# kubeai-project/kubeai

Measured on AMD Instinct MI355X. Metric: output_tokens_per_s (k6 multi-turn chat), higher is better.
Workload: dtype fp8; 1 GPU; model=llama-3-8b, global_batch=40, seq_len=8192, parallelism=dp1, prefix_cache=True

## Files before the change

kubeai_amd/csrc/bindings.cpp:

```cpp
#include <torch/extension.h>

#include <utility>

#include "attention_plan.h"

void rmsnorm(torch::Tensor out, torch::Tensor x, torch::Tensor weight,
             double eps);
void fused_add_rmsnorm(torch::Tensor x, torch::Tensor residual,
                       torch::Tensor weight, double eps);
void rope(torch::Tensor q, torch::Tensor k, torch::Tensor positions,
          torch::Tensor cos_sin);
void rope_and_cache(torch::Tensor q, torch::Tensor k, torch::Tensor v,
                    torch::Tensor positions, torch::Tensor cos_sin,
                    torch::Tensor k_cache, torch::Tensor v_cache,
                    torch::Tensor slot_mapping);
void reshape_and_cache(torch::Tensor k, torch::Tensor v, torch::Tensor k_cache,
                       torch::Tensor v_cache, torch::Tensor slot_mapping);
void paged_attention_decode(torch::Tensor out, torch::Tensor q,
                            torch::Tensor k_cache, torch::Tensor v_cache,
                            torch::Tensor block_tables, torch::Tensor seq_lens,
                            double scale, int64_t window, double softcap);
void paged_attention_decode_fp8(torch::Tensor out, torch::Tensor out_fp8,
                                torch::Tensor out_scale, torch::Tensor q,
                                torch::Tensor k_cache, torch::Tensor v_cache,
// ... 14 lines not shown
                             torch::Tensor seq_lens, double scale,
                             int64_t window, double softcap);
void silu_and_mul(torch::Tensor out, torch::Tensor x);
void gelu_and_mul(torch::Tensor out, torch::Tensor x);
void skinny_gemm(torch::Tensor y, torch::Tensor x, torch::Tensor w);
void int4_dequant(torch::Tensor out, torch::Tensor qp, torch::Tensor sp,
                  torch::Tensor zp, int64_t N, int64_t K, int64_t group);
void int4_gemm(torch::Tensor y, torch::Tensor x, torch::Tensor qp,
               torch::Tensor sp, torch::Tensor zp, int64_t N, int64_t K,
               int64_t group);
int64_t int4_gemm_tiles(int64_t N, int64_t M);
void greedy_sample(torch::Tensor out, torch::Tensor logits);
void gumbel_sample(torch::Tensor out, torch::Tensor logits,
                   torch::Tensor temperature, torch::Tensor seeds,
                   int64_t step);
void sgmv(torch::Tensor y, torch::Tensor x, torch::Tensor A, torch::Tensor B,
          torch::Tensor idx, double scale);
void register_chwbl(pybind11::module_& m);
pybind11::bytes xgmi_alloc();
void xgmi_connect(int64_t rank, int64_t world,
                  const std::vector<pybind11::bytes>& handles);
void xgmi_fused_allreduce_add_rmsnorm(torch::Tensor x, torch::Tensor residual,
                                      torch::Tensor weight, double eps);
int64_t xgmi_error_count();
int64_t xgmi_max_elems();
void xgmi_shutdown();
void rmsnorm_fp8(torch::Tensor out, torch::Tensor out_scale, torch::Tensor x,
                 torch::Tensor weight, double eps);
void fused_add_rmsnorm_fp8(torch::Tensor out, torch::Tensor out_scale,
                           torch::Tensor x, torch::Tensor residual,
                           torch::Tensor weight, double eps);
void silu_and_mul_fp8(torch::Tensor out, torch::Tensor out_scale,
                      torch::Tensor x);
void quant_fp8(torch::Tensor out, torch::Tensor out_scale, torch::Tensor x);
void nucleus_stats(torch::Tensor m, torch::Tensor z, torch::Tensor logits,
                   torch::Tensor temps);
void nucleus_accept(torch::Tensor ok, torch::Tensor logits,
                    torch::Tensor cand, torch::Tensor m, torch::Tensor z,
                    torch::Tensor temps, torch::Tensor top_ps,
                    torch::Tensor top_ks);

static std::pair<int64_t, int64_t> prefill_plan(int64_t Tq, int64_t B,
                                                int64_t n_q, int64_t n_kv,
                                                int64_t hd, int64_t max_blocks,
                                                int64_t window,
                                                double softcap) {
  TORCH_CHECK(n_kv > 0 && n_q % n_kv == 0);
  const attn_plan::PrefillPlan p = attn_plan::prefill_plan(
      Tq, (int)B, (int)n_q, (int)n_kv, (int)hd, (int)max_blocks, window,
// ... 32 lines not shown
        "decode attention kernel (q, k, v are only read)");
  m.def("paged_attention_prefill", &paged_attention_prefill,
        "paged causal flash attention over cached KV");
  m.def("gelu_and_mul", &gelu_and_mul, "GeGLU tanh-gelu(gate)*up");
  m.def("silu_and_mul", &silu_and_mul, "SwiGLU activation");
  m.def("skinny_gemm", &skinny_gemm, "weight-streaming GEMM for M<=64");
  m.def("int4_dequant", &int4_dequant,
        "packed int4 weight -> bf16 [N, K], bit-equal to Int4Weight.dequant()");
  m.def("int4_gemm", &int4_gemm,
        "fused dequant + GEMM over a packed int4 weight, M <= 64");
  m.def("int4_gemm_tiles", &int4_gemm_tiles,
        "16-column tiles per workgroup int4_gemm launches with",
        pybind11::arg("N"), pybind11::arg("M"));
  m.def("greedy_sample", &greedy_sample, "argmax sampling");
  m.def("gumbel_sample", &gumbel_sample, "temperature sampling (hash RNG)");
  m.def("rmsnorm_fp8", &rmsnorm_fp8, "rmsnorm with fused fp8 row quant");
  m.def("fused_add_rmsnorm_fp8", &fused_add_rmsnorm_fp8,
        "residual add + rmsnorm with fused fp8 row quant");
  m.def("silu_and_mul_fp8", &silu_and_mul_fp8, "SwiGLU with fused fp8 quant");
  m.def("quant_fp8", &quant_fp8, "bf16 -> fp8 row quant");
  m.def("nucleus_stats", &nucleus_stats, "per-row softmax max + Z");
  m.def("nucleus_accept", &nucleus_accept,
        "nucleus membership of sampled tokens (mass above < p, rank < k)");
  m.def("xgmi_alloc", &xgmi_alloc, "allocate + export the IPC comm buffer");
  m.def("xgmi_connect", &xgmi_connect, "open peer IPC buffers");
  m.def("xgmi_fused_allreduce_add_rmsnorm", &xgmi_fused_allreduce_add_rmsnorm,
        "one-shot xGMI all-reduce fused with residual add + RMSNorm");
  m.def("xgmi_error_count", &xgmi_error_count, "spin-wait timeout count");
  m.def("xgmi_max_elems", &xgmi_max_elems, "one-shot capacity (bf16 elems)");
  m.def("xgmi_shutdown", &xgmi_shutdown, "free/close comm buffers");
  m.def("sgmv", &sgmv, "segmented gather LoRA apply (one adapter segment)");
  register_chwbl(m);
}
```

kubeai_amd/csrc/common.h:

```cpp
#pragma once

#include <hip/hip_runtime.h>
#include <hip/hip_bf16.h>
#include <hip/hip_fp16.h>
#include <hip/hip_fp8.h>
#include <stdint.h>
#include <c10/hip/HIPStream.h>

#define WAVE_SIZE 64
#define DEV_INLINE __device__ __forceinline__

typedef __hip_bfloat16 bf16_t;

typedef ushort __attribute__((ext_vector_type(8))) ushort8;
typedef ushort __attribute__((ext_vector_type(4))) ushort4_t;
typedef float __attribute__((ext_vector_type(4))) float4_t;

DEV_INLINE float bf16_to_f32(ushort u) {
  union {
    uint32_t i;
    float f;
  } c;
  c.i = ((uint32_t)u) << 16;
  return c.f;
// ... 126 lines not shown
#pragma unroll
  for (int j = 0; j < 4; ++j) {
    packed[j].x = f32_to_fp8(f[2 * j] * inv_scale);
    packed[j].y = f32_to_fp8(f[2 * j + 1] * inv_scale);
  }
  return *reinterpret_cast<uint2*>(packed);
}

DEV_INLINE float row_scale_fp8(const float amax, float* smem,
                               float* __restrict__ scale_out) {
  const float gmax = fmaxf(block_amax(amax, smem), 1e-6f);
  if (threadIdx.x == 0) *scale_out = gmax / 448.0f;
  return 448.0f / gmax;
}

DEV_INLINE float silu(const float x) { return x / (1.0f + __expf(-x)); }

DEV_INLINE uint64_t splitmix64(uint64_t z) {
  z += 0x9e3779b97f4a7c15ull;
  z = (z ^ (z >> 30)) * 0xbf58476d1ce4e5b9ull;
  z = (z ^ (z >> 27)) * 0x94d049bb133111ebull;
  return z ^ (z >> 31);
}

DEV_INLINE float hash_uniform(uint64_t key, uint64_t idx) {
  uint64_t h = splitmix64(key ^ (idx * 0xd1342543de82ef95ull));
  uint32_t m = (uint32_t)(h >> 40);
  return ((float)m + 1.0f) * (1.0f / 16777216.0f);
}

// ... 9 lines not shown
```

kubeai_amd/csrc/row_kernels.hip:

```cpp
#include <torch/extension.h>

#include <type_traits>

#include "common.h"
#include "dispatch.h"

namespace {

constexpr int kBlock = 256;
constexpr int kBlockWide = 512;
constexpr int kMaxIters = 8;
constexpr int kMaxH = kBlockWide * 8 * kMaxIters;

template <int kThreads, int kIters>
DEV_INLINE void store_row_fp8(unsigned char* __restrict__ orow,
                              const float (&vals)[kIters][8],
                              const float inv_scale, const int nvec) {
#pragma unroll
  for (int it = 0; it < kIters; ++it) {
    const int i = threadIdx.x + it * kThreads;
    if (i < nvec)
      *reinterpret_cast<uint2*>(orow + i * 8) = quant8_fp8(vals[it], inv_scale);
  }
}

template <bool kFused, bool kFp8Out, int kThreads, int kIters>
__launch_bounds__(kThreads) __global__ void rmsnorm_kernel(
    std::conditional_t<kFp8Out, unsigned char, ushort>* __restrict__ out,
    float* __restrict__ out_scale,
    ushort* __restrict__ x,
    ushort* __restrict__ residual,
    const ushort* __restrict__ w,
    const float eps, const int H) {
  const int row = blockIdx.x;
  ushort8* xrow = reinterpret_cast<ushort8*>(x + (int64_t)row * H);
  ushort8* rrow =
      kFused ? reinterpret_cast<ushort8*>(residual + (int64_t)row * H) : nullptr;
// ... 77 lines not shown
    for (int j = 0; j < 8; ++j) v[j] = bf16_to_f32(xv[j]);
  }
};

struct LoadSwiglu {
  static constexpr int kInWidth = 2;
  DEV_INLINE static void load(const ushort* __restrict__ in, const int W,
                              const int i, float (&v)[8]) {
    const ushort8 g = reinterpret_cast<const ushort8*>(in)[i];
    const ushort8 u = reinterpret_cast<const ushort8*>(in + W)[i];
#pragma unroll
    for (int j = 0; j < 8; ++j) v[j] = silu(bf16_to_f32(g[j])) * bf16_to_f32(u[j]);
  }
};

template <typename Producer, int kThreads, int kIters>
__launch_bounds__(kThreads) __global__ void row_fp8_kernel(
    unsigned char* __restrict__ out,
    float* __restrict__ out_scale,
    const ushort* __restrict__ xin,
    const int W) {
  const int row = blockIdx.x;
  const ushort* in = xin + (int64_t)row * Producer::kInWidth * W;
  const int nvec = W / 8;

  float vals[kIters][8];
  float amax = 0.f;
#pragma unroll
  for (int it = 0; it < kIters; ++it) {
    const int i = threadIdx.x + it * kThreads;
    if (i < nvec) {
      Producer::load(in, W, i, vals[it]);
#pragma unroll
      for (int j = 0; j < 8; ++j) amax = fmaxf(amax, fabsf(vals[it][j]));
    }
  }
  __shared__ float red[16];
  const float inv_scale = row_scale_fp8(amax, red, out_scale + row);
  store_row_fp8<kThreads, kIters>(out + (int64_t)row * W, vals, inv_scale, nvec);
}

enum class RowPolicy { kNorm, kMax };

template <RowPolicy kPolicy, typename Launch>
void dispatch_row(const int nvec, Launch&& launch) {
  if (nvec <= kBlock) {
    launch(Int<kBlock>{}, Int<1>{});
  } else if (nvec <= kBlock * 2) {
    launch(Int<kBlock>{}, Int<2>{});
  } else if (nvec <= kBlock * 4) {
    launch(Int<kBlock>{}, Int<4>{});
  } else if constexpr (kPolicy == RowPolicy::kNorm) {
    if (nvec <= kBlock * kMaxIters) launch(Int<kBlock>{}, Int<kMaxIters>{});
    else launch(Int<kBlockWide>{}, Int<kMaxIters>{});
// ... 16 lines not shown
  check_row_op(x, H);
  const int T = x.numel() / H;
  using out_t = std::conditional_t<kFp8Out, unsigned char, ushort>;
  dispatch_row<RowPolicy::kNorm>(H / 8, [&](auto threads, auto iters) {
    constexpr int kThreads = decltype(threads)::value;
    constexpr int kIters = decltype(iters)::value;
    hipLaunchKernelGGL((rmsnorm_kernel<kFused, kFp8Out, kThreads, kIters>),
                       dim3(T), dim3(kThreads), 0,
                       c10::hip::getCurrentHIPStream().stream(), (out_t*)out,
                       out_scale, (ushort*)x.data_ptr(), (ushort*)residual,
                       (const ushort*)weight.data_ptr(), (float)eps, H);
  });
  HIP_CHECK_KERNEL();
}

template <typename Producer>
void launch_row_fp8(torch::Tensor& out, torch::Tensor& out_scale,
                    const torch::Tensor& x) {
  const int W = x.size(-1) / Producer::kInWidth;
  check_row_op(x, W);
  TORCH_CHECK(x.size(-1) == (int64_t)W * Producer::kInWidth);
  const int T = x.numel() / x.size(-1);
  if (T == 0) return;
  dispatch_row<RowPolicy::kMax>(W / 8, [&](auto threads, auto iters) {
    constexpr int kThreads = decltype(threads)::value;
    constexpr int kIters = decltype(iters)::value;
    hipLaunchKernelGGL((row_fp8_kernel<Producer, kThreads, kIters>), dim3(T),
                       dim3(kThreads), 0,
                       c10::hip::getCurrentHIPStream().stream(),
                       (unsigned char*)out.data_ptr(),
                       out_scale.data_ptr<float>(),
                       (const ushort*)x.data_ptr(), W);
  });
  HIP_CHECK_KERNEL();
}

}

void rmsnorm(torch::Tensor out, torch::Tensor x, torch::Tensor weight,
             double eps) {
  TORCH_CHECK(out.is_contiguous());
  launch_rmsnorm<false, false>(out.data_ptr(), nullptr, x, nullptr, weight, eps);
// ... 16 lines not shown
                           torch::Tensor x, torch::Tensor residual,
                           torch::Tensor weight, double eps) {
  TORCH_CHECK(residual.is_contiguous());
  launch_rmsnorm<true, true>(out.data_ptr(), out_scale.data_ptr<float>(), x,
                             residual.data_ptr(), weight, eps);
}

void silu_and_mul_fp8(torch::Tensor out, torch::Tensor out_scale,
                      torch::Tensor x) {
  launch_row_fp8<LoadSwiglu>(out, out_scale, x);
}

void quant_fp8(torch::Tensor out, torch::Tensor out_scale, torch::Tensor x) {
  launch_row_fp8<LoadBf16>(out, out_scale, x);
}
```

kubeai_amd/csrc/sampling.hip:

```cpp
#include <torch/extension.h>

#include "common.h"

namespace {

constexpr int kBlock = 256;
constexpr int kSplits = 32;

template <bool kGumbel>
__global__ void sample_stage1(
    float* __restrict__ part_val,
    int32_t* __restrict__ part_idx,
    const float* __restrict__ logits,
    const float* __restrict__ temperature,
    const int64_t* __restrict__ seeds,
    const int64_t step, const int V) {
  const int b = blockIdx.x;
  const int split = blockIdx.y;
  const int chunk = (V + kSplits - 1) / kSplits;
  const int lo = split * chunk;
  const int hi = min(V, lo + chunk);
  const float* row = logits + (int64_t)b * V;
  float temp = 1.0f;
  uint64_t key = 0;
  bool greedy = !kGumbel;
  if constexpr (kGumbel) {
    temp = temperature[b];
    if (temp <= 0.f) greedy = true;
    key = (uint64_t)seeds[b] * 1000003ull + (uint64_t)step;
  }

  float best = -INFINITY;
  int best_idx = V;
  for (int v = lo + threadIdx.x; v < hi; v += kBlock) {
    float val = row[v];
    if (!greedy) {
      float u = hash_uniform(key, (uint64_t)v);
      val = val / temp + (-__logf(-__logf(u)));
    }
    if (val > best || (val == best && v < best_idx)) {
      best = val;
      best_idx = v;
    }
  }
#pragma unroll
  for (int off = 32; off > 0; off >>= 1) {
    float ov = __shfl_xor(best, off, 64);
    int oi = __shfl_xor(best_idx, off, 64);
    if (ov > best || (ov == best && oi < best_idx)) {
      best = ov;
      best_idx = oi;
    }
  }
  __shared__ float sval[4];
  __shared__ int sidx[4];
  const int wave = threadIdx.x / WAVE_SIZE;
  if (threadIdx.x % WAVE_SIZE == 0) {
    sval[wave] = best;
    sidx[wave] = best_idx;
  }
  __syncthreads();
  if (threadIdx.x == 0) {
#pragma unroll
    for (int w = 1; w < kBlock / WAVE_SIZE; ++w) {
      if (sval[w] > best || (sval[w] == best && sidx[w] < best_idx)) {
        best = sval[w];
        best_idx = sidx[w];
      }
    }
    part_val[b * kSplits + split] = best;
    part_idx[b * kSplits + split] = best_idx;
  }
}

__global__ void sample_stage2(int64_t* __restrict__ out,
                              const float* __restrict__ part_val,
                              const int32_t* __restrict__ part_idx) {
  const int b = blockIdx.x;
  const int lane = threadIdx.x;
  float best = (lane < kSplits) ? part_val[b * kSplits + lane] : -INFINITY;
  int best_idx = (lane < kSplits) ? part_idx[b * kSplits + lane] : INT32_MAX;
#pragma unroll
  for (int off = 32; off > 0; off >>= 1) {
    float ov = __shfl_xor(best, off, 64);
    int oi = __shfl_xor(best_idx, off, 64);
    if (ov > best || (ov == best && oi < best_idx)) {
      best = ov;
      best_idx = oi;
    }
  }
  if (lane == 0) out[b] = best_idx;
}

template <bool kGumbel>
void launch_sample(torch::Tensor out, torch::Tensor logits,
                   const float* temp_ptr, const int64_t* seed_ptr,
                   int64_t step) {
  const int B = logits.size(0), V = logits.size(1);
  if (B == 0) return;
  auto opts = torch::TensorOptions().device(logits.device());
  auto part_val = torch::empty({B, kSplits}, opts.dtype(torch::kFloat32));
  auto part_idx = torch::empty({B, kSplits}, opts.dtype(torch::kInt32));
  auto stream = c10::hip::getCurrentHIPStream().stream();
  hipLaunchKernelGGL((sample_stage1<kGumbel>), dim3(B, kSplits), dim3(kBlock),
                     0, stream, part_val.data_ptr<float>(),
                     part_idx.data_ptr<int32_t>(), logits.data_ptr<float>(),
                     temp_ptr, seed_ptr, step, V);
  HIP_CHECK_KERNEL();
  hipLaunchKernelGGL(sample_stage2, dim3(B), dim3(WAVE_SIZE), 0, stream,
                     out.data_ptr<int64_t>(), part_val.data_ptr<float>(),
                     part_idx.data_ptr<int32_t>());
  HIP_CHECK_KERNEL();
}

}

void greedy_sample(torch::Tensor out, torch::Tensor logits) {
  TORCH_CHECK(logits.is_contiguous());
  TORCH_CHECK(logits.scalar_type() == torch::kFloat32,
              "sampling expects fp32 logits");
  launch_sample<false>(out, logits, nullptr, nullptr, 0);
}

void gumbel_sample(torch::Tensor out, torch::Tensor logits,
                   torch::Tensor temperature, torch::Tensor seeds,
                   int64_t step) {
  TORCH_CHECK(logits.is_contiguous());
  TORCH_CHECK(logits.scalar_type() == torch::kFloat32);
  TORCH_CHECK(temperature.scalar_type() == torch::kFloat32);
  TORCH_CHECK(seeds.scalar_type() == torch::kInt64);
  launch_sample<true>(out, logits, temperature.data_ptr<float>(),
                      seeds.data_ptr<int64_t>(), step);
}


namespace {

__global__ void nucleus_stats_kernel(
    float* __restrict__ m_out, float* __restrict__ z_out,
    const float* __restrict__ logits, const float* __restrict__ temps,
    const int V) {
  const int row = blockIdx.x;
  const float* x = logits + (int64_t)row * V;
  const float t = fmaxf(temps[row], 1e-6f);
  __shared__ float red[16];
  float m = -INFINITY;
  for (int i = threadIdx.x; i < V; i += blockDim.x) m = fmaxf(m, x[i]);
// ... 88 lines not shown
```

kubeai_amd/engine/quant.py:

```python
from __future__ import annotations

import torch
import torch.nn as nn

FP8_DTYPE = torch.float8_e4m3fn
FP8_MAX = 448.0


class Fp8Linear(nn.Module):

    def __init__(self, weight_bf16: torch.Tensor, bias: torch.Tensor | None = None):
        super().__init__()
        if bias is not None:
            self.register_buffer("bias", bias.detach().to(torch.bfloat16))
        else:
            self.bias = None
        w = weight_bf16.detach().float()
        w_amax = w.abs().amax(dim=1, keepdim=True).clamp_min(1e-6)
        w_scale = w_amax / FP8_MAX
        wq = (w / w_scale).clamp(-FP8_MAX, FP8_MAX).to(FP8_DTYPE)
        self.register_buffer("weight_fp8", wq.contiguous())
        self.register_buffer("weight_scale", w_scale.reshape(1, -1).contiguous())
        self.out_features, self.in_features = weight_bf16.shape

# ... 7 lines not shown
        if not xq.is_cuda:
            x = xq.float() * x_scale.view(-1, 1)
            w = self.weight_fp8.float() * self.weight_scale.reshape(-1, 1)
            y = (x @ w.t()).to(torch.bfloat16)
            return y + self.bias if self.bias is not None else y
        return torch._scaled_mm(
            xq,
            self.weight_fp8.t(),
            scale_a=x_scale.view(-1, 1),
            scale_b=self.weight_scale,
            bias=self.bias,
            out_dtype=torch.bfloat16,
        )

    def forward(self, x: torch.Tensor) -> torch.Tensor:
        a_amax = x.float().abs().amax(dim=-1, keepdim=True).clamp_min(1e-6)
        a_scale = a_amax / FP8_MAX
        xq = (x.float() / a_scale).clamp(-FP8_MAX, FP8_MAX).to(FP8_DTYPE)
        if not x.is_cuda:
            return self.forward_quantized(xq, a_scale.squeeze(-1))
        return torch._scaled_mm(
            xq,
            self.weight_fp8.t(),
            scale_a=a_scale,
            scale_b=self.weight_scale,
            bias=self.bias,
            out_dtype=torch.bfloat16,
        )


_TARGETS = ("qkv_proj", "o_proj", "gate_up_proj", "down_proj", "lm_head")


# ... 19 lines not shown
```

kubeai_amd/engine/runner.py:

```python
from __future__ import annotations

import os
from typing import Optional

import torch

from kubeai_amd import ops
from kubeai_amd.models.config import ModelArchConfig
from kubeai_amd.models.llama import LlamaForCausalLM

from .batch import ForwardBatch
from .scheduler import SchedulerOutput


class _DecodeGraph:

    def __init__(self, runner: "ModelRunner", b_pad: int, bt_max: int):
        dev = runner.device
        self.b_pad = b_pad
        self.bt_max = bt_max
        self.input_ids = torch.zeros(b_pad, dtype=torch.int32, device=dev)
        self.positions = torch.zeros(b_pad, dtype=torch.int32, device=dev)
        self.slots = torch.full((b_pad,), -1, dtype=torch.int64, device=dev)
        self.block_tables = torch.zeros(
            (b_pad, bt_max), dtype=torch.int32, device=dev
        )
        self.seq_lens = torch.ones(b_pad, dtype=torch.int32, device=dev)
        logits_idx = torch.arange(b_pad, dtype=torch.int64, device=dev)
        self.fb = ForwardBatch(
            input_ids=self.input_ids,
            positions=self.positions,
            slot_mapping=self.slots,
            n_decode=b_pad,
            decode_block_tables=self.block_tables,
            decode_seq_lens=self.seq_lens,
            n_prefill=0,
            prefill_query_start_loc=None,
            prefill_seq_lens=None,
            prefill_block_tables=None,
            logits_indices=logits_idx,
        )
        torch.cuda.synchronize()
        for _ in range(2):
            h = runner.model(self.fb)
            runner.model.compute_logits(h[logits_idx])
        torch.cuda.synchronize()
        self.graph = torch.cuda.CUDAGraph()
        with torch.cuda.graph(self.graph):
            h = runner.model(self.fb)
            self.logits = runner.model.compute_logits(h[logits_idx])

    def run(self, input_ids, positions, slots, tables, seq_lens) -> torch.Tensor:
        b = len(input_ids)
        self.input_ids[:b].copy_(input_ids, non_blocking=True)
        self.positions[:b].copy_(positions, non_blocking=True)
        self.slots[:b].copy_(slots, non_blocking=True)
        if b < self.b_pad:
            self.slots[b:].fill_(-1)
            self.seq_lens[b:].fill_(1)
            self.block_tables[b:].fill_(0)
        self.block_tables[:b, : tables.shape[1]].copy_(tables, non_blocking=True)
        if tables.shape[1] < self.bt_max:
            self.block_tables[:b, tables.shape[1] :].fill_(0)
        self.seq_lens[:b].copy_(seq_lens, non_blocking=True)
        self.graph.replay()
        return self.logits[:b]


class ModelRunner:
    def __init__(
        self,
        arch: ModelArchConfig,
        device: str = "cuda",
        dtype: torch.dtype = torch.bfloat16,
        block_size: int = 16,
        num_gpu_blocks: Optional[int] = None,
        gpu_memory_utilization: float = 0.90,
        seed: int = 0,
        tp_group=None,
# ... 286 lines not shown
            self._graphs[b_pad] = g
        bs = self.block_size
        ids, pos, slots, lens = [], [], [], []
        import numpy as np

        tables = np.zeros((b, g.bt_max), dtype=np.int32)
        for i, ss in enumerate(out.decode):
            req = ss.req
            t = ss.chunk_start
            ids.append(req.tokens[t])
            pos.append(t)
            slots.append(req.block_table[t // bs] * bs + t % bs)
            lens.append(t + 1)
            bt = req.block_table
            tables[i, : len(bt)] = bt
        return g.run(
            torch.tensor(ids, dtype=torch.int32),
            torch.tensor(pos, dtype=torch.int32),
            torch.tensor(slots, dtype=torch.int64),
            torch.from_numpy(tables),
            torch.tensor(lens, dtype=torch.int32),
        )

    @torch.inference_mode()
    def execute(self, out: SchedulerOutput, step: int) -> dict[str, int]:
        logits = None
        if (
            self.enable_graphs
            and not out.prefill
            and out.decode
            and not (
                getattr(self, "lora_manager", None) is not None
                and self.lora_manager.active
            )
        ):
            logits = self._execute_graph(out)
        if logits is None:
# ... 35 lines not shown
            if r.params.logit_bias:
                for t, b in r.params.logit_bias.items():
                    if 0 <= t < V:
                        rows.append(i)
                        cols.append(t)
                        vals.append(b)
        if rows:
            flat = torch.tensor(
                [ri * V + ci for ri, ci in zip(rows, cols)],
                dtype=torch.int64, device=dev_l,
            )
            logits.view(-1).scatter_add_(
                0, flat, torch.tensor(vals, dtype=logits.dtype, device=dev_l)
            )
        temps = [r.params.temperature for r in sample_reqs]
        if all(t <= 0.0 for t in temps):
            tokens = ops.greedy_sample(logits.contiguous())
        else:
            needs_topk = any(
                (r.params.top_p < 1.0 or r.params.top_k > 0)
                and r.params.temperature > 0
                for r in sample_reqs
            )
            dev = self.device
            t_t = torch.tensor(temps, dtype=torch.float32, device=dev)
            seeds = torch.tensor(
                [
                    r.params.seed if r.params.seed is not None else _seed_of(r.request_id)
                    for r in sample_reqs
                ],
                dtype=torch.int64,
                device=dev,
            )
            if needs_topk:
                tokens = _sample_topk_topp(
                    logits,
                    [r.params.top_p for r in sample_reqs],
                    [r.params.top_k for r in sample_reqs],
                    [r.params.temperature for r in sample_reqs],
                    t_t, seeds, step,
                    cache=self._sampling_cache,
                ).to(dev)
            else:
                tokens = ops.gumbel_sample(logits.contiguous(), t_t, seeds, step)
        tokens = tokens.cpu().tolist()
        if any(r.params.json_mode for r in sample_reqs):
            tokens = self._constrain_json(sample_reqs, tokens, logits)
        tokens_t = torch.tensor(tokens, dtype=torch.int64, device=logits.device)
        lse = torch.logsumexp(logits, dim=-1)
        chosen = logits.gather(1, tokens_t.view(-1, 1)).squeeze(1)
        logprobs = (chosen - lse).cpu().tolist()
        self.last_logprobs = {
            r.request_id: float(lp) for r, lp in zip(sample_reqs, logprobs)
        }
        self.last_top_logprobs = {}
        want = max((r.params.logprobs for r in sample_reqs), default=0)
        if want > 0:
            k = min(want, logits.shape[-1])
            tv, ti = (logits - lse.unsqueeze(1)).topk(k, dim=-1)
            tv, ti = tv.cpu().tolist(), ti.cpu().tolist()
            for r, vs, ids in zip(sample_reqs, tv, ti):
                if r.params.logprobs > 0:
                    n = r.params.logprobs
                    self.last_top_logprobs[r.request_id] = [
                        (int(i), float(v)) for i, v in zip(ids[:n], vs[:n])
                    ]
# ... 217 lines not shown
```

kubeai_amd/ops/__init__.py:

```python
from __future__ import annotations

import os

import torch

from . import ref

_C = None
_C_IMPORT_ERROR: Exception | None = None
try:
    from kubeai_amd import _C
except Exception as e:
    _C_IMPORT_ERROR = e


def have_hip_ext() -> bool:
    return _C is not None


def _require_ext() -> None:
    if _C is None:
        raise RuntimeError(
            "kubeai_amd HIP extension (kubeai_amd._C) is not built but a GPU "
            "tensor reached the ops layer. Build it with "
# ... 275 lines not shown
    T, two_i = x.shape
    out, scale = _empty_fp8_rows((T, two_i // 2), x.device)
    _C.silu_and_mul_fp8(out, scale, x)
    return out, scale


def quant_fp8(x):
    if not x.is_cuda:
        return ref.quant_fp8(x)
    _require_ext()
    out, scale = _empty_fp8_rows(x.shape, x.device)
    _C.quant_fp8(out, scale, x)
    return out, scale


def greedy_sample(logits):
    if logits.is_cuda:
        _require_ext()
        out = torch.empty(logits.shape[0], dtype=torch.int64, device=logits.device)
        _C.greedy_sample(out, logits)
        return out
    return ref.greedy_sample(logits)


def gumbel_sample(logits, temperature, seeds, step: int):
    if logits.is_cuda:
        _require_ext()
        out = torch.empty(logits.shape[0], dtype=torch.int64, device=logits.device)
        _C.gumbel_sample(out, logits, temperature, seeds, step)
        return out
    return ref.gumbel_sample(logits, temperature, seeds, step)


def nucleus_stats(logits, temps):
    if logits.is_cuda:
        _require_ext()
        S = logits.shape[0]
        m = torch.empty(S, dtype=torch.float32, device=logits.device)
        z = torch.empty_like(m)
        _C.nucleus_stats(m, z, logits, temps)
        return m, z
    t = temps.clamp_min(1e-6).unsqueeze(1)
    m = logits.max(dim=-1).values
    z = torch.exp((logits - m.unsqueeze(1)) / t).sum(-1)
    return m, z

# ... 16 lines not shown
```

kubeai_amd/ops/ref.py:

```python
from __future__ import annotations

import math

import torch



def rmsnorm(x: torch.Tensor, weight: torch.Tensor, eps: float) -> torch.Tensor:
    xf = x.float()
    var = xf.pow(2).mean(dim=-1, keepdim=True)
    y = xf * torch.rsqrt(var + eps) * weight.float()
    return y.to(x.dtype)


def fused_add_rmsnorm(
    x: torch.Tensor, residual: torch.Tensor, weight: torch.Tensor, eps: float
) -> tuple[torch.Tensor, torch.Tensor]:
    res = (x.float() + residual.float())
    y = rmsnorm(res, weight, eps)
    return y.to(x.dtype), res.to(x.dtype)



def make_cos_sin_cache(
# ... 227 lines not shown
    B, V = lf.shape
    out = torch.empty(B, dtype=torch.int64, device=logits.device)
    idx = torch.arange(V)
    for b in range(B):
        t = float(temperature[b])
        if t <= 0.0:
            out[b] = int(lf[b].argmax())
            continue
        key = (int(seeds[b]) * 1000003 + step) & _U64
        u = hash_uniform(key, idx).to(lf.device)
        g = -torch.log(-torch.log(u))
        out[b] = int((lf[b] / t + g).argmax())
    return out


def topk_topp_sample(
    logits: torch.Tensor,
    temperature: torch.Tensor,
    top_p: torch.Tensor,
    top_k: torch.Tensor,
    seeds: torch.Tensor,
    step: int,
) -> torch.Tensor:
    lf = logits.float()
    B, V = lf.shape
    out = torch.empty(B, dtype=torch.int64, device=logits.device)
    for b in range(B):
        t = float(temperature[b])
        if t <= 0.0:
            out[b] = int(lf[b].argmax())
# ... 9 lines not shown
        sp, si = sp[keep], si[keep]
        gen = torch.Generator(device="cpu")
        gen.manual_seed(int(seeds[b]) * 1000003 + step)
        r = float(torch.rand((), generator=gen)) * float(sp.sum())
        idx = int(torch.searchsorted(sp.cumsum(0), torch.tensor(r)).clamp(max=sp.shape[0] - 1))
        out[b] = int(si[idx])
    return out


def quant_fp8(x: torch.Tensor):
    xf = x.float()
    amax = xf.abs().amax(dim=-1).clamp_min(1e-6)
    scale = amax / 448.0
    q = (xf / scale[:, None]).clamp(-448.0, 448.0).to(torch.float8_e4m3fn)
    return q, scale
```

Before: 7380 tok/s.

## Fuse sampling with logprob/logsumexp, add div-form fp8 quant kernel, stage graph inputs

Sampling kernels now also compute the row logsumexp and the chosen token's logprob, so the separate torch logsumexp, gather and extra device-to-host copy after sampling are gone. Tokens and logprobs are packed into one buffer and copied to the host together. A division-form fp8 row-quant kernel is added for Fp8Linear, and the decode graph inputs are staged through a pinned host buffer with a single copy. These cut per-step launches and host syncs, at the cost of more kernel variants and added complexity.

```diff
diff --git a/kubeai_amd/csrc/bindings.cpp b/kubeai_amd/csrc/bindings.cpp
--- a/kubeai_amd/csrc/bindings.cpp
+++ b/kubeai_amd/csrc/bindings.cpp
@@ -52,6 +52,14 @@
 void gumbel_sample(torch::Tensor out, torch::Tensor logits,
                    torch::Tensor temperature, torch::Tensor seeds,
                    int64_t step);
+void greedy_sample_logprob(torch::Tensor out, torch::Tensor out_logprob,
+                           torch::Tensor out_lse, torch::Tensor logits);
+void gumbel_sample_logprob(torch::Tensor out, torch::Tensor out_logprob,
+                           torch::Tensor out_lse, torch::Tensor logits,
+                           torch::Tensor temperature, torch::Tensor seeds,
+                           int64_t step);
+void token_logprobs(torch::Tensor out_logprob, torch::Tensor out_lse,
+                    torch::Tensor logits, torch::Tensor tokens);
 void sgmv(torch::Tensor y, torch::Tensor x, torch::Tensor A, torch::Tensor B,
           torch::Tensor idx, double scale);
 void register_chwbl(pybind11::module_& m);
@@ -71,6 +79,8 @@
 void silu_and_mul_fp8(torch::Tensor out, torch::Tensor out_scale,
                       torch::Tensor x);
 void quant_fp8(torch::Tensor out, torch::Tensor out_scale, torch::Tensor x);
+void quant_fp8_div(torch::Tensor out, torch::Tensor out_scale,
+                   torch::Tensor x);
 void nucleus_stats(torch::Tensor m, torch::Tensor z, torch::Tensor logits,
                    torch::Tensor temps);
 void nucleus_accept(torch::Tensor ok, torch::Tensor logits,
@@ -133,11 +143,19 @@
         pybind11::arg("N"), pybind11::arg("M"));
   m.def("greedy_sample", &greedy_sample, "argmax sampling");
   m.def("gumbel_sample", &gumbel_sample, "temperature sampling (hash RNG)");
+  m.def("greedy_sample_logprob", &greedy_sample_logprob,
+        "argmax sampling + the token's logprob and the row logsumexp");
+  m.def("gumbel_sample_logprob", &gumbel_sample_logprob,
+        "temperature sampling + the token's logprob and the row logsumexp");
+  m.def("token_logprobs", &token_logprobs,
+        "logprob of given tokens and the row logsumexp, one launch");
   m.def("rmsnorm_fp8", &rmsnorm_fp8, "rmsnorm with fused fp8 row quant");
   m.def("fused_add_rmsnorm_fp8", &fused_add_rmsnorm_fp8,
         "residual add + rmsnorm with fused fp8 row quant");
   m.def("silu_and_mul_fp8", &silu_and_mul_fp8, "SwiGLU with fused fp8 quant");
   m.def("quant_fp8", &quant_fp8, "bf16 -> fp8 row quant");
+  m.def("quant_fp8_div", &quant_fp8_div,
+        "bf16 -> fp8 row quant, division form (Fp8Linear.forward)");
   m.def("nucleus_stats", &nucleus_stats, "per-row softmax max + Z");
   m.def("nucleus_accept", &nucleus_accept,
         "nucleus membership of sampled tokens (mass above < p, rank < k)");
diff --git a/kubeai_amd/csrc/common.h b/kubeai_amd/csrc/common.h
--- a/kubeai_amd/csrc/common.h
+++ b/kubeai_amd/csrc/common.h
@@ -164,6 +164,26 @@
   return 448.0f / gmax;
 }
 
+DEV_INLINE float row_scale_fp8_div(const float amax, float* smem,
+                                   float* __restrict__ scale_out) {
+  const float gmax = fmaxf(block_amax(amax, smem), 1e-6f);
+  const float scale = gmax * (float)(1.0 / 448.0);
+  if (threadIdx.x == 0) *scale_out = scale;
+  return scale;
+}
+
+DEV_INLINE uint2 quant8_fp8_div(const float (&f)[8], const float scale) {
+  uchar2 packed[4];
+#pragma unroll
+  for (int j = 0; j < 4; ++j) {
+    packed[j].x =
+        f32_to_fp8(fminf(fmaxf(f[2 * j] / scale, -448.0f), 448.0f));
+    packed[j].y =
+        f32_to_fp8(fminf(fmaxf(f[2 * j + 1] / scale, -448.0f), 448.0f));
+  }
+  return *reinterpret_cast<uint2*>(packed);
+}
+
 DEV_INLINE float silu(const float x) { return x / (1.0f + __expf(-x)); }
 
 DEV_INLINE uint64_t splitmix64(uint64_t z) {
diff --git a/kubeai_amd/csrc/row_kernels.hip b/kubeai_amd/csrc/row_kernels.hip
--- a/kubeai_amd/csrc/row_kernels.hip
+++ b/kubeai_amd/csrc/row_kernels.hip
@@ -12,15 +12,16 @@
 constexpr int kMaxIters = 8;
 constexpr int kMaxH = kBlockWide * 8 * kMaxIters;
 
-template <int kThreads, int kIters>
+template <int kThreads, int kIters, bool kDiv = false>
 DEV_INLINE void store_row_fp8(unsigned char* __restrict__ orow,
                               const float (&vals)[kIters][8],
-                              const float inv_scale, const int nvec) {
+                              const float factor, const int nvec) {
 #pragma unroll
   for (int it = 0; it < kIters; ++it) {
     const int i = threadIdx.x + it * kThreads;
     if (i < nvec)
-      *reinterpret_cast<uint2*>(orow + i * 8) = quant8_fp8(vals[it], inv_scale);
+      *reinterpret_cast<uint2*>(orow + i * 8) =
+          kDiv ? quant8_fp8_div(vals[it], factor) : quant8_fp8(vals[it], factor);
   }
 }
 
@@ -128,7 +129,7 @@
   }
 };
 
-template <typename Producer, int kThreads, int kIters>
+template <typename Producer, bool kDiv, int kThreads, int kIters>
 __launch_bounds__(kThreads) __global__ void row_fp8_kernel(
     unsigned char* __restrict__ out,
     float* __restrict__ out_scale,
@@ -150,8 +151,10 @@
     }
   }
   __shared__ float red[16];
-  const float inv_scale = row_scale_fp8(amax, red, out_scale + row);
-  store_row_fp8<kThreads, kIters>(out + (int64_t)row * W, vals, inv_scale, nvec);
+  const float factor = kDiv ? row_scale_fp8_div(amax, red, out_scale + row)
+                            : row_scale_fp8(amax, red, out_scale + row);
+  store_row_fp8<kThreads, kIters, kDiv>(out + (int64_t)row * W, vals, factor,
+                                        nvec);
 }
 
 enum class RowPolicy { kNorm, kMax };
@@ -198,7 +201,7 @@
   HIP_CHECK_KERNEL();
 }
 
-template <typename Producer>
+template <typename Producer, bool kDiv = false>
 void launch_row_fp8(torch::Tensor& out, torch::Tensor& out_scale,
                     const torch::Tensor& x) {
   const int W = x.size(-1) / Producer::kInWidth;
@@ -209,7 +212,7 @@
   dispatch_row<RowPolicy::kMax>(W / 8, [&](auto threads, auto iters) {
     constexpr int kThreads = decltype(threads)::value;
     constexpr int kIters = decltype(iters)::value;
-    hipLaunchKernelGGL((row_fp8_kernel<Producer, kThreads, kIters>), dim3(T),
+    hipLaunchKernelGGL((row_fp8_kernel<Producer, kDiv, kThreads, kIters>), dim3(T),
                        dim3(kThreads), 0,
                        c10::hip::getCurrentHIPStream().stream(),
                        (unsigned char*)out.data_ptr(),
@@ -256,3 +259,8 @@
 void quant_fp8(torch::Tensor out, torch::Tensor out_scale, torch::Tensor x) {
   launch_row_fp8<LoadBf16>(out, out_scale, x);
 }
+
+void quant_fp8_div(torch::Tensor out, torch::Tensor out_scale,
+                   torch::Tensor x) {
+  launch_row_fp8<LoadBf16, true>(out, out_scale, x);
+}
diff --git a/kubeai_amd/csrc/sampling.hip b/kubeai_amd/csrc/sampling.hip
--- a/kubeai_amd/csrc/sampling.hip
+++ b/kubeai_amd/csrc/sampling.hip
@@ -1,20 +1,50 @@
 #include <torch/extension.h>
 
 #include "common.h"
+#include "dispatch.h"
 
 namespace {
 
 constexpr int kBlock = 256;
+constexpr int kWaves = kBlock / WAVE_SIZE;
 constexpr int kSplits = 32;
-
-template <bool kGumbel>
-__global__ void sample_stage1(
-    float* __restrict__ part_val,
-    int32_t* __restrict__ part_idx,
+constexpr int kRegIters = 16;
+
+DEV_INLINE float max_waves(const float (&s)[kWaves]) {
+  return fmaxf(fmaxf(s[0], s[1]), fmaxf(s[2], s[3]));
+}
+
+DEV_INLINE float sum_waves(const float (&s)[kWaves]) {
+  return ((s[0] + s[1]) + s[2]) + s[3];
+}
+static_assert(kWaves == 4, "max_waves / sum_waves spell four waves");
+
+DEV_INLINE float exp_ref(const float m) { return m == -INFINITY ? 0.f : m; }
+
+DEV_INLINE float merge_lse(const float m, const float s) {
+  const float M = wave_reduce_max(m);
+  const float t = (m == -INFINITY) ? 0.f : s * expf(m - M);
+  float S = 0.f;
+#pragma unroll
+  for (int i = 0; i < kSplits; ++i) S += __shfl(t, i, 64);
+  return logf(S) + M;
+}
+
+struct SamplePartials {
+  float* val;
+  int32_t* idx;
+  float* m;
+  float* s;
+};
+
+template <bool kGumbel, bool kLse, bool kRegs>
+__launch_bounds__(kBlock) __global__ void sample_stage1(
+    const SamplePartials part,
     const float* __restrict__ logits,
     const float* __restrict__ temperature,
     const int64_t* __restrict__ seeds,
     const int64_t step, const int V) {
+  static_assert(kLse || !kRegs, "registers serve the second sweep only");
   const int b = blockIdx.x;
   const int split = blockIdx.y;
   const int chunk = (V + kSplits - 1) / kSplits;
@@ -32,8 +62,9 @@
 
   float best = -INFINITY;
   int best_idx = V;
-  for (int v = lo + threadIdx.x; v < hi; v += kBlock) {
-    float val = row[v];
+  float m = -INFINITY;
+  auto visit = [&](const int v, const float raw) {
+    float val = raw;
     if (!greedy) {
       float u = hash_uniform(key, (uint64_t)v);
       val = val / temp + (-__logf(-__logf(u)));
@@ -42,6 +73,22 @@
       best = val;
       best_idx = v;
     }
+    if constexpr (kLse) m = fmaxf(m, raw);
+  };
+  float x[kRegs ? kRegIters : 1];
+  if constexpr (kRegs) {
+#pragma unroll
+    for (int it = 0; it < kRegIters; ++it) {
+      const int v = lo + threadIdx.x + it * kBlock;
+      x[it] = v < hi ? row[v] : -INFINITY;
+    }
+#pragma unroll
+    for (int it = 0; it < kRegIters; ++it) {
+      const int v = lo + threadIdx.x + it * kBlock;
+      if (v < hi) visit(v, x[it]);
+    }
+  } else {
+    for (int v = lo + threadIdx.x; v < hi; v += kBlock) visit(v, row[v]);
   }
 #pragma unroll
   for (int off = 32; off > 0; off >>= 1) {
@@ -52,34 +99,64 @@
       best_idx = oi;
     }
   }
-  __shared__ float sval[4];
-  __shared__ int sidx[4];
+  if constexpr (kLse) m = wave_reduce_max(m);
+  __shared__ float sval[kWaves];
+  __shared__ int sidx[kWaves];
+  __shared__ float smax[kWaves];
+  __shared__ float ssum[kWaves];
   const int wave = threadIdx.x / WAVE_SIZE;
   if (threadIdx.x % WAVE_SIZE == 0) {
     sval[wave] = best;
     sidx[wave] = best_idx;
+    if constexpr (kLse) smax[wave] = m;
   }
   __syncthreads();
   if (threadIdx.x == 0) {
 #pragma unroll
-    for (int w = 1; w < kBlock / WAVE_SIZE; ++w) {
+    for (int w = 1; w < kWaves; ++w) {
       if (sval[w] > best || (sval[w] == best && sidx[w] < best_idx)) {
         best = sval[w];
         best_idx = sidx[w];
       }
     }
-    part_val[b * kSplits + split] = best;
-    part_idx[b * kSplits + split] = best_idx;
-  }
-}
-
+    part.val[b * kSplits + split] = best;
+    part.idx[b * kSplits + split] = best_idx;
+  }
+  if constexpr (kLse) {
+    m = max_waves(smax);
+    const float ref = exp_ref(m);
+    float s = 0.f;
+    if constexpr (kRegs) {
+#pragma unroll
+      for (int it = 0; it < kRegIters; ++it) {
+        const int v = lo + threadIdx.x + it * kBlock;
+        if (v < hi) s += expf(x[it] - ref);
+      }
+    } else {
+      for (int v = lo + threadIdx.x; v < hi; v += kBlock)
+        s += expf(row[v] - ref);
+    }
+    s = wave_reduce_sum(s);
+    if (threadIdx.x % WAVE_SIZE == 0) ssum[wave] = s;
+    __syncthreads();
+    if (threadIdx.x == 0) {
+      part.m[b * kSplits + split] = m;
+      part.s[b * kSplits + split] = sum_waves(ssum);
+    }
+  }
+}
+
+template <bool kLse>
 __global__ void sample_stage2(int64_t* __restrict__ out,
-                              const float* __restrict__ part_val,
-                              const int32_t* __restrict__ part_idx) {
+                              float* __restrict__ out_logprob,
+                              float* __restrict__ out_lse,
+                              const SamplePartials part,
+                              const float* __restrict__ logits,
+                              const int V) {
   const int b = blockIdx.x;
   const int lane = threadIdx.x;
-  float best = (lane < kSplits) ? part_val[b * kSplits + lane] : -INFINITY;
-  int best_idx = (lane < kSplits) ? part_idx[b * kSplits + lane] : INT32_MAX;
+  float best = (lane < kSplits) ? part.val[b * kSplits + lane] : -INFINITY;
+  int best_idx = (lane < kSplits) ? part.idx[b * kSplits + lane] : INT32_MAX;
 #pragma unroll
   for (int off = 32; off > 0; off >>= 1) {
     float ov = __shfl_xor(best, off, 64);
@@ -89,48 +166,178 @@
       best_idx = oi;
     }
   }
+  if constexpr (kLse) {
+    const float lse =
+        merge_lse((lane < kSplits) ? part.m[b * kSplits + lane] : -INFINITY,
+                  (lane < kSplits) ? part.s[b * kSplits + lane] : 0.f);
+    if (lane == 0) {
+      const float xt =
+          best_idx < V ? logits[(int64_t)b * V + best_idx] : (float)NAN;
+      out_logprob[b] = xt - lse;
+      out_lse[b] = lse;
+    }
+  }
   if (lane == 0) out[b] = best_idx;
 }
 
-template <bool kGumbel>
-void launch_sample(torch::Tensor out, torch::Tensor logits,
-                   const float* temp_ptr, const int64_t* seed_ptr,
-                   int64_t step) {
+constexpr int kGroups = 4;
+static_assert(kSplits % kGroups == 0, "every group runs every round");
+
+__launch_bounds__(kBlock* kGroups) __global__ void token_logprobs_kernel(
+    float* __restrict__ out_logprob,
+    float* __restrict__ out_lse,
+    const float* __restrict__ logits,
+    const int64_t* __restrict__ tokens,
+    const int V) {
+  const int b = blockIdx.x;
+  const int g = threadIdx.x / kBlock;
+  const int tid = threadIdx.x % kBlock;
+  const int wave = tid / WAVE_SIZE;
+  const float* row = logits + (int64_t)b * V;
+  const int chunk = (V + kSplits - 1) / kSplits;
+  __shared__ float smax[kGroups][kWaves];
+  __shared__ float ssum[kGroups][kWaves];
+  __shared__ float pm[kSplits];
+  __shared__ float ps[kSplits];
+  for (int r = 0; r < kSplits / kGroups; ++r) {
+    const int split = r * kGroups + g;
+    const int lo = split * chunk;
+    const int hi = min(V, lo + chunk);
+    float m = -INFINITY;
+    for (int v = lo + tid; v < hi; v += kBlock) m = fmaxf(m, row[v]);
+    m = wave_reduce_max(m);
+    if (tid % WAVE_SIZE == 0) smax[g][wave] = m;
+    __syncthreads();
+    m = max_waves(smax[g]);
+    const float ref = exp_ref(m);
+    float s = 0.f;
+    for (int v = lo + tid; v < hi; v += kBlock) s += expf(row[v] - ref);
+    s = wave_reduce_sum(s);
+    if (tid % WAVE_SIZE == 0) ssum[g][wave] = s;
+    __syncthreads();
+    if (tid == 0) {
+      pm[split] = m;
+      ps[split] = sum_waves(ssum[g]);
+    }
+  }
+  __syncthreads();
+  if (threadIdx.x < WAVE_SIZE) {
+    const int lane = threadIdx.x;
+    const float lse = merge_lse((lane < kSplits) ? pm[lane] : -INFINITY,
+                                (lane < kSplits) ? ps[lane] : 0.f);
+    if (lane == 0) {
+      const int64_t t = tokens[b];
+      const float xt = (t >= 0 && t < V) ? row[t] : (float)NAN;
+      out_logprob[b] = xt - lse;
+      out_lse[b] = lse;
+    }
+  }
+}
+
+void check_logits(const torch::Tensor& logits) {
+  TORCH_CHECK(logits.dim() == 2 && logits.is_contiguous());
+  TORCH_CHECK(logits.scalar_type() == torch::kFloat32,
+              "sampling expects fp32 logits");
+}
+
+template <typename T>
+T* row_output(const torch::Tensor& t, const torch::Tensor& logits) {
+  TORCH_CHECK(t.is_contiguous() && t.numel() == logits.size(0) &&
+              t.device() == logits.device());
+  return t.data_ptr<T>();
+}
+
+template <bool kGumbel, bool kLse>
+void launch_sample(int64_t* out, float* out_logprob, float* out_lse,
+                   const torch::Tensor& logits, const float* temp_ptr,
+                   const int64_t* seed_ptr, int64_t step) {
   const int B = logits.size(0), V = logits.size(1);
   if (B == 0) return;
-  auto opts = torch::TensorOptions().device(logits.device());
-  auto part_val = torch::empty({B, kSplits}, opts.dtype(torch::kFloat32));
-  auto part_idx = torch::empty({B, kSplits}, opts.dtype(torch::kInt32));
+  const int64_t n = (int64_t)B * kSplits;
+  auto buf = torch::empty(
+      {(kLse ? 4 : 2) * n},
+      torch::TensorOptions().device(logits.device()).dtype(torch::kInt32));
+  int32_t* w = buf.data_ptr<int32_t>();
+  const SamplePartials part{reinterpret_cast<float*>(w), w + n,
+                            kLse ? reinterpret_cast<float*>(w + 2 * n) : nullptr,
+                            kLse ? reinterpret_cast<float*>(w + 3 * n) : nullptr};
   auto stream = c10::hip::getCurrentHIPStream().stream();
-  hipLaunchKernelGGL((sample_stage1<kGumbel>), dim3(B, kSplits), dim3(kBlock),
-                     0, stream, part_val.data_ptr<float>(),
-                     part_idx.data_ptr<int32_t>(), logits.data_ptr<float>(),
-                     temp_ptr, seed_ptr, step, V);
+  const int chunk = (V + kSplits - 1) / kSplits;
+  dispatch_bool(kLse && chunk <= kBlock * kRegIters, [&](auto regs) {
+    constexpr bool kRegs = kLse && decltype(regs)::value;
+    hipLaunchKernelGGL((sample_stage1<kGumbel, kLse, kRegs>),
+                       dim3(B, kSplits), dim3(kBlock), 0, stream, part,
+                       logits.data_ptr<float>(), temp_ptr, seed_ptr, step, V);
+  });
   HIP_CHECK_KERNEL();
-  hipLaunchKernelGGL(sample_stage2, dim3(B), dim3(WAVE_SIZE), 0, stream,
-                     out.data_ptr<int64_t>(), part_val.data_ptr<float>(),
-                     part_idx.data_ptr<int32_t>());
+  hipLaunchKernelGGL(sample_stage2<kLse>, dim3(B), dim3(WAVE_SIZE), 0, stream,
+                     out, out_logprob, out_lse, part, logits.data_ptr<float>(),
+                     V);
   HIP_CHECK_KERNEL();
 }
 
+void check_gumbel(const torch::Tensor& logits, const torch::Tensor& temperature,
+                  const torch::Tensor& seeds) {
+  TORCH_CHECK(temperature.scalar_type() == torch::kFloat32);
+  TORCH_CHECK(seeds.scalar_type() == torch::kInt64);
+  TORCH_CHECK(temperature.is_contiguous() && seeds.is_contiguous());
+  TORCH_CHECK(temperature.numel() == logits.size(0) &&
+              seeds.numel() == logits.size(0));
+}
+
 }
 
 void greedy_sample(torch::Tensor out, torch::Tensor logits) {
-  TORCH_CHECK(logits.is_contiguous());
-  TORCH_CHECK(logits.scalar_type() == torch::kFloat32,
-              "sampling expects fp32 logits");
-  launch_sample<false>(out, logits, nullptr, nullptr, 0);
+  check_logits(logits);
+  launch_sample<false, false>(row_output<int64_t>(out, logits), nullptr,
+                              nullptr, logits, nullptr, nullptr, 0);
 }
 
 void gumbel_sample(torch::Tensor out, torch::Tensor logits,
                    torch::Tensor temperature, torch::Tensor seeds,
                    int64_t step) {
-  TORCH_CHECK(logits.is_contiguous());
-  TORCH_CHECK(logits.scalar_type() == torch::kFloat32);
-  TORCH_CHECK(temperature.scalar_type() == torch::kFloat32);
-  TORCH_CHECK(seeds.scalar_type() == torch::kInt64);
-  launch_sample<true>(out, logits, temperature.data_ptr<float>(),
-                      seeds.data_ptr<int64_t>(), step);
+  check_logits(logits);
+  check_gumbel(logits, temperature, seeds);
+  launch_sample<true, false>(row_output<int64_t>(out, logits), nullptr, nullptr,
+                             logits, temperature.data_ptr<float>(),
+                             seeds.data_ptr<int64_t>(), step);
+}
+
+void greedy_sample_logprob(torch::Tensor out, torch::Tensor out_logprob,
+                           torch::Tensor out_lse, torch::Tensor logits) {
+  check_logits(logits);
+  launch_sample<false, true>(row_output<int64_t>(out, logits),
+                             row_output<float>(out_logprob, logits),
+                             row_output<float>(out_lse, logits), logits,
+                             nullptr, nullptr, 0);
+}
+
+void gumbel_sample_logprob(torch::Tensor out, torch::Tensor out_logprob,
+                           torch::Tensor out_lse, torch::Tensor logits,
+                           torch::Tensor temperature, torch::Tensor seeds,
+                           int64_t step) {
+  check_logits(logits);
+  check_gumbel(logits, temperature, seeds);
+  launch_sample<true, true>(row_output<int64_t>(out, logits),
+                            row_output<float>(out_logprob, logits),
+                            row_output<float>(out_lse, logits), logits,
+                            temperature.data_ptr<float>(),
+                            seeds.data_ptr<int64_t>(), step);
+}
+
+void token_logprobs(torch::Tensor out_logprob, torch::Tensor out_lse,
+                    torch::Tensor logits, torch::Tensor tokens) {
+  check_logits(logits);
+  TORCH_CHECK(tokens.scalar_type() == torch::kInt64);
+  const int B = logits.size(0), V = logits.size(1);
+  float* lp = row_output<float>(out_logprob, logits);
+  float* lse = row_output<float>(out_lse, logits);
+  const int64_t* tok = row_output<int64_t>(tokens, logits);
+  if (B == 0) return;
+  hipLaunchKernelGGL(token_logprobs_kernel, dim3(B), dim3(kBlock * kGroups), 0,
+                     c10::hip::getCurrentHIPStream().stream(), lp, lse,
+                     logits.data_ptr<float>(), tok, V);
+  HIP_CHECK_KERNEL();
 }
 
 
diff --git a/kubeai_amd/engine/quant.py b/kubeai_amd/engine/quant.py
--- a/kubeai_amd/engine/quant.py
+++ b/kubeai_amd/engine/quant.py
@@ -2,6 +2,8 @@
 
 import torch
 import torch.nn as nn
+
+from kubeai_amd import ops
 
 FP8_DTYPE = torch.float8_e4m3fn
 FP8_MAX = 448.0
@@ -45,9 +47,7 @@
         )
 
     def forward(self, x: torch.Tensor) -> torch.Tensor:
-        a_amax = x.float().abs().amax(dim=-1, keepdim=True).clamp_min(1e-6)
-        a_scale = a_amax / FP8_MAX
-        xq = (x.float() / a_scale).clamp(-FP8_MAX, FP8_MAX).to(FP8_DTYPE)
+        xq, a_scale = ops.quant_fp8_div(x)
         if not x.is_cuda:
             return self.forward_quantized(xq, a_scale.squeeze(-1))
         return torch._scaled_mm(
diff --git a/kubeai_amd/engine/runner.py b/kubeai_amd/engine/runner.py
--- a/kubeai_amd/engine/runner.py
+++ b/kubeai_amd/engine/runner.py
@@ -15,17 +15,33 @@
 
 class _DecodeGraph:
 
+    @staticmethod
+    def _carve(buf, n: int, bt_max: int, i64):
+        return (
+            buf[2 * n : 3 * n],
+            buf[3 * n : 4 * n],
+            buf[: 2 * n].view(i64),
+            buf[5 * n :].reshape(n, bt_max),
+            buf[4 * n : 5 * n],
+        )
+
     def __init__(self, runner: "ModelRunner", b_pad: int, bt_max: int):
+        import numpy as np
+
         dev = runner.device
         self.b_pad = b_pad
         self.bt_max = bt_max
-        self.input_ids = torch.zeros(b_pad, dtype=torch.int32, device=dev)
-        self.positions = torch.zeros(b_pad, dtype=torch.int32, device=dev)
-        self.slots = torch.full((b_pad,), -1, dtype=torch.int64, device=dev)
-        self.block_tables = torch.zeros(
-            (b_pad, bt_max), dtype=torch.int32, device=dev
-        )
-        self.seq_lens = torch.ones(b_pad, dtype=torch.int32, device=dev)
+        self.staged = os.environ.get("KUBEAI_GRAPH_STAGED_INPUTS", "1") != "0"
+        words = b_pad * (5 + bt_max)
+        self._host = torch.zeros(words, dtype=torch.int32, pin_memory=True)
+        self._host_views = self._carve(self._host.numpy(), b_pad, bt_max, np.int64)
+        self._host_views[2][:] = -1
+        self._host_views[4][:] = 1
+        self._dev = self._host.to(dev)
+        (
+            self.input_ids, self.positions, self.slots, self.block_tables,
+            self.seq_lens,
+        ) = self._carve(self._dev, b_pad, bt_max, torch.int64)
         logits_idx = torch.arange(b_pad, dtype=torch.int64, device=dev)
         self.fb = ForwardBatch(
             input_ids=self.input_ids,
@@ -52,9 +68,30 @@
 
     def run(self, input_ids, positions, slots, tables, seq_lens) -> torch.Tensor:
         b = len(input_ids)
-        self.input_ids[:b].copy_(input_ids, non_blocking=True)
-        self.positions[:b].copy_(positions, non_blocking=True)
-        self.slots[:b].copy_(slots, non_blocking=True)
+        if not self.staged:
+            return self._run_unstaged(input_ids, positions, slots, tables, seq_lens)
+        h_ids, h_pos, h_slots, h_tables, h_lens = self._host_views
+        h_ids[:b], h_ids[b:] = input_ids, 0
+        h_pos[:b], h_pos[b:] = positions, 0
+        h_slots[:b], h_slots[b:] = slots, -1
+        h_lens[:b], h_lens[b:] = seq_lens, 1
+        w = tables.shape[1]
+        h_tables[:b, :w] = tables
+        h_tables[:b, w:] = 0
+        h_tables[b:] = 0
+        self._dev.copy_(self._host, non_blocking=True)
+        self.graph.replay()
+        return self.logits[:b]
+
+    def _run_unstaged(self, input_ids, positions, slots, tables, seq_lens):
+        b = len(input_ids)
+        tables = torch.from_numpy(tables)
+        i32 = lambda x: torch.tensor(x, dtype=torch.int32)
+        self.input_ids[:b].copy_(i32(input_ids), non_blocking=True)
+        self.positions[:b].copy_(i32(positions), non_blocking=True)
+        self.slots[:b].copy_(
+            torch.tensor(slots, dtype=torch.int64), non_blocking=True
+        )
         if b < self.b_pad:
             self.slots[b:].fill_(-1)
             self.seq_lens[b:].fill_(1)
@@ -62,7 +99,7 @@
         self.block_tables[:b, : tables.shape[1]].copy_(tables, non_blocking=True)
         if tables.shape[1] < self.bt_max:
             self.block_tables[:b, tables.shape[1] :].fill_(0)
-        self.seq_lens[:b].copy_(seq_lens, non_blocking=True)
+        self.seq_lens[:b].copy_(i32(seq_lens), non_blocking=True)
         self.graph.replay()
         return self.logits[:b]
 
@@ -379,13 +416,7 @@
             lens.append(t + 1)
             bt = req.block_table
             tables[i, : len(bt)] = bt
-        return g.run(
-            torch.tensor(ids, dtype=torch.int32),
-            torch.tensor(pos, dtype=torch.int32),
-            torch.tensor(slots, dtype=torch.int64),
-            torch.from_numpy(tables),
-            torch.tensor(lens, dtype=torch.int32),
-        )
+        return g.run(ids, pos, slots, tables, lens)
 
     @torch.inference_mode()
     def execute(self, out: SchedulerOutput, step: int) -> dict[str, int]:
@@ -451,8 +482,11 @@
                 0, flat, torch.tensor(vals, dtype=logits.dtype, device=dev_l)
             )
         temps = [r.params.temperature for r in sample_reqs]
+        logits = logits.contiguous()
         if all(t <= 0.0 for t in temps):
-            tokens = ops.greedy_sample(logits.contiguous())
+            res = ops.greedy_sample_logprob(logits)
+            lse = res.lse
+            tokens, logprobs = ops.sample_to_host(res)
         else:
             needs_topk = any(
                 (r.params.top_p < 1.0 or r.params.top_k > 0)
@@ -470,7 +504,7 @@
                 device=dev,
             )
             if needs_topk:
-                tokens = _sample_topk_topp(
+                tokens_t = _sample_topk_topp(
                     logits,
                     [r.params.top_p for r in sample_reqs],
                     [r.params.top_k for r in sample_reqs],
@@ -478,15 +512,27 @@
                     t_t, seeds, step,
                     cache=self._sampling_cache,
                 ).to(dev)
+                lp_t, lse = ops.token_logprobs(logits, tokens_t)
+                tokens = tokens_t.cpu().tolist()
+                logprobs = lp_t.cpu().tolist()
             else:
-                tokens = ops.gumbel_sample(logits.contiguous(), t_t, seeds, step)
-        tokens = tokens.cpu().tolist()
+                res = ops.gumbel_sample_logprob(logits, t_t, seeds, step)
+                lse = res.lse
+                tokens, logprobs = ops.sample_to_host(res)
         if any(r.params.json_mode for r in sample_reqs):
+            sampled = list(tokens)
             tokens = self._constrain_json(sample_reqs, tokens, logits)
-        tokens_t = torch.tensor(tokens, dtype=torch.int64, device=logits.device)
-        lse = torch.logsumexp(logits, dim=-1)
-        chosen = logits.gather(1, tokens_t.view(-1, 1)).squeeze(1)
-        logprobs = (chosen - lse).cpu().tolist()
+            moved = [i for i, (a, b) in enumerate(zip(sampled, tokens)) if a != b]
+            if moved:
+                lp_t, _ = ops.token_logprobs(
+                    logits[torch.tensor(moved, device=logits.device)],
+                    torch.tensor(
+                        [tokens[i] for i in moved],
+                        dtype=torch.int64, device=logits.device,
+                    ),
+                )
+                for i, lp in zip(moved, lp_t.cpu().tolist()):
+                    logprobs[i] = lp
         self.last_logprobs = {
             r.request_id: float(lp) for r, lp in zip(sample_reqs, logprobs)
         }
diff --git a/kubeai_amd/ops/__init__.py b/kubeai_amd/ops/__init__.py
--- a/kubeai_amd/ops/__init__.py
+++ b/kubeai_amd/ops/__init__.py
@@ -1,6 +1,7 @@
 from __future__ import annotations
 
 import os
+from typing import NamedTuple
 
 import torch
 
@@ -313,6 +314,26 @@
     return out, scale
 
 
+_QUANT_DIV_MAX_H = 32768
+
+
+def quant_fp8_div(x):
+    if (
+        x.is_cuda
+        and x.dtype == torch.bfloat16
+        and x.dim() == 2
+        and x.is_contiguous()
+        and x.shape[1] % 8 == 0
+        and 0 < x.shape[1] <= _QUANT_DIV_MAX_H
+        and os.environ.get("KUBEAI_QUANT_DIV_KERNEL", "1") != "0"
+    ):
+        _require_ext()
+        out, scale = _empty_fp8_rows(x.shape, x.device)
+        _C.quant_fp8_div(out, scale, x)
+        return out, scale.view(-1, 1)
+    return ref.quant_fp8_div(x)
+
+
 def greedy_sample(logits):
     if logits.is_cuda:
         _require_ext()
@@ -329,6 +350,61 @@
         _C.gumbel_sample(out, logits, temperature, seeds, step)
         return out
     return ref.gumbel_sample(logits, temperature, seeds, step)
+
+
+class SampleResult(NamedTuple):
+
+    tokens: torch.Tensor
+    logprob: torch.Tensor
+    lse: torch.Tensor
+    packed: torch.Tensor | None = None
+
+
+def _empty_sample_result(logits) -> SampleResult:
+    B = logits.shape[0]
+    packed = torch.empty(2 * B, dtype=torch.int64, device=logits.device)
+    f = packed[B:].view(torch.float32)
+    return SampleResult(packed[:B], f[:B], f[B:], packed)
+
+
+def sample_to_host(res: SampleResult) -> tuple[list[int], list[float]]:
+    if res.packed is None or not res.packed.is_cuda:
+        return res.tokens.tolist(), res.logprob.tolist()
+    B = res.tokens.shape[0]
+    host = res.packed[: B + (B + 1) // 2].cpu()
+    return host[:B].tolist(), host[B:].view(torch.float32)[:B].tolist()
+
+
+def greedy_sample_logprob(logits) -> SampleResult:
+    if logits.is_cuda:
+        _require_ext()
+        res = _empty_sample_result(logits)
+        _C.greedy_sample_logprob(res.tokens, res.logprob, res.lse, logits)
+        return res
+    return SampleResult(*ref.greedy_sample_logprob(logits))
+
+
+def gumbel_sample_logprob(logits, temperature, seeds, step: int) -> SampleResult:
+    if logits.is_cuda:
+        _require_ext()
+        res = _empty_sample_result(logits)
+        _C.gumbel_sample_logprob(
+            res.tokens, res.logprob, res.lse, logits, temperature, seeds, step
+        )
+        return res
+    return SampleResult(
+        *ref.gumbel_sample_logprob(logits, temperature, seeds, step)
+    )
+
+
+def token_logprobs(logits, tokens):
+    if logits.is_cuda:
+        _require_ext()
+        B = logits.shape[0]
+        out = torch.empty((2, B), dtype=torch.float32, device=logits.device)
+        _C.token_logprobs(out[0], out[1], logits, tokens)
+        return out[0], out[1]
+    return ref.token_logprobs(logits, tokens)
 
 
 def nucleus_stats(logits, temps):
diff --git a/kubeai_amd/ops/ref.py b/kubeai_amd/ops/ref.py
--- a/kubeai_amd/ops/ref.py
+++ b/kubeai_amd/ops/ref.py
@@ -265,6 +265,25 @@
     return out
 
 
+def token_logprobs(
+    logits: torch.Tensor,
+    tokens: torch.Tensor,
+) -> tuple[torch.Tensor, torch.Tensor]:
+    lse = torch.logsumexp(logits, dim=-1)
+    chosen = logits.gather(1, tokens.view(-1, 1)).squeeze(1)
+    return chosen - lse, lse
+
+
+def greedy_sample_logprob(logits: torch.Tensor):
+    tokens = greedy_sample(logits)
+    return (tokens, *token_logprobs(logits, tokens))
+
+
+def gumbel_sample_logprob(logits, temperature, seeds, step: int):
+    tokens = gumbel_sample(logits, temperature, seeds, step)
+    return (tokens, *token_logprobs(logits, tokens))
+
+
 def topk_topp_sample(
     logits: torch.Tensor,
     temperature: torch.Tensor,
@@ -304,3 +323,10 @@
     scale = amax / 448.0
     q = (xf / scale[:, None]).clamp(-448.0, 448.0).to(torch.float8_e4m3fn)
     return q, scale
+
+
+def quant_fp8_div(x: torch.Tensor):
+    amax = x.float().abs().amax(dim=-1, keepdim=True).clamp_min(1e-6)
+    scale = amax / 448.0
+    q = (x.float() / scale).clamp(-448.0, 448.0).to(torch.float8_e4m3fn)
+    return q, scale
```

After: 7624 tok/s (median of 6 runs). +3.3%, better.
